# kanster/moped

Hardware: AMD Instinct MI355X
Metric: detections/sec (frames/s) 640x480 ~3k SIFT vs N models (higher is better)
Workload: dtype f32

## Files before the change

### include/moped_hip.h

```cpp
#ifndef MOPED_HIP_H
#define MOPED_HIP_H

#include <stddef.h>
#include <stdint.h>

#ifdef __cplusplus
extern "C" {
#endif

#define MH_DESC_DIM 128
#define MH_MAX_BATCH 32
#define MH_MAX_IMAGES 8
#define MH_MAX_MODELS 8192
#define MH_OK 0
#define MH_ERR_ARG (-1)
#define MH_ERR_HIP (-2)
#define MH_ERR_CAPACITY (-3)
#define MH_ERR_NODEVICE (-4)

typedef struct mh_ctx mh_ctx;


int mh_create(int device, mh_ctx** out);
void mh_destroy(mh_ctx* ctx);
// ... 35 lines not shown
int mh_match_stats(mh_ctx* ctx, int Q, uint32_t stats[4], int reset);
int mh_match_set_mode(mh_ctx* ctx, int mode);
int mh_pose_set_split(mh_ctx* ctx, int on);
int mh_match_launches(mh_ctx* ctx, uint32_t out[3]);
float mh_screen_margin(float qq, float dmax);
int mh_screen_values(mh_ctx* ctx, const float* q_host, int Q, int n_rows, float* out_host, float* dmax, float* spread,
                     int shape );
uint16_t mh_screen_record_value(float top, float thr);
void mh_screen_record_bounds(uint16_t value_bits, uint32_t row0, float tau, float spread, int N, float dmax, float* lo,
                             float* hi);
float mh_screen_pack_value(float v, uint32_t id, int bits);
float mh_screen_pack_pert(float qq, float dmax, int bits);
void mh_screen_sample_bounds(uint16_t value_bits, float tau, float pert, float dmax, float* lo, float* hi);
void mh_screen_launch_plan(int Q, int q_expected, int N, int32_t out[8]);
int mh_match_incomplete(mh_ctx* ctx, uint32_t* count, int reset);
int mh_screen_sample_values(mh_ctx* ctx, const float* q_host, int Q, const int32_t* row0_host, float* out_host);
int mh_match_query_candidates(mh_ctx* ctx, int Q, uint32_t* out);

int mh_match_local_dev(mh_ctx* ctx, const float* qn_dev, const float* qnorm_dev, int Q,
                       int32_t* idx1_dev, float* d1_dev, float* d2_dev);
int mh_match_local_counted_dev(mh_ctx* ctx, const float* qn_dev, const float* qnorm_dev, int Q,
                               const int32_t* q_count_dev, int q_expected, int32_t* idx1_dev, float* d1_dev,
                               float* d2_dev);
int mh_match_merge_dev(mh_ctx* ctx, const int32_t* idx1_s_dev, const float* d1_s_dev,
                       const float* d2_s_dev, int n_shards, int Q,
                       int32_t* idx1_dev, float* d1_dev, float* d2_dev);
int mh_normalize_dev(mh_ctx* ctx, float* q_dev, float* qnorm_dev, int Q);


int mh_meanshift(mh_ctx* ctx, const float* pts_host, int n, int dim, float radius,
// ... 387 lines not shown
```

### moped_amd/capi.py

```python
from __future__ import annotations

import ctypes as C
import os

import numpy as np

_HERE = os.path.dirname(os.path.abspath(__file__))
LIB_PATH = os.environ.get("MH_LIB_PATH") or os.path.join(_HERE, "libmoped_hip.so")

MH_OK = 0
MH_ERR_CAPACITY = -3


class MhError(RuntimeError):
    pass


class mh_corr(C.Structure):
    _fields_ = [("u", C.c_float), ("v", C.c_float), ("x", C.c_float), ("y", C.c_float), ("z", C.c_float)]


class mh_cam(C.Structure):
    _fields_ = [("K", C.c_float * 4), ("cam", C.c_float * 7)]

# ... 113 lines not shown
    "mh_db_upload_raw", "mh_db_share", "mh_match_stats", "mh_match_set_mode", "mh_match_launches", "mh_pose_set_split", "mh_frame_fetch_match_points", "mh_screen_margin", "mh_frame_counters", "mh_match_timing", "mh_frame_set_images", "mh_filter_images",
    "mh_pose_ransac_images",
    "mh_comm_unique_id", "mh_comm_create", "mh_comm_create_all", "mh_comm_create_host", "mh_comm_destroy", "mh_comm_info",
    "mh_frame_enqueue_sharded", "mh_frame_enqueue_sharded_batch", "mh_frame_enqueue_sharded_all",
    "mh_frame_previous_objects", "mh_frame_gather_objects", "mh_frame_enqueue_batch", "mh_frame_set_depth_image_batch",
    "mh_pose_kernel_info", "mh_db_upload_blocks", "mh_frame_fetch_matches_slot", "mh_frame_fetch_match_reps_slot",
    "mh_screen_values", "mh_screen_record_value", "mh_screen_record_bounds", "mh_reserve_batch", "mh_frame_run_host",
    "mh_frame_block_stride", "mh_frame_fetch_batch_async", "mh_frame_fetch_previous_async", "mh_frame_fetch_wait",
    "mh_frame_fetch_query", "mh_host_alloc", "mh_host_free", "mh_frame_run_host_begin", "mh_frame_wait_descriptors",
    "mh_step_match", "mh_step_match_fetch", "mh_step_cluster", "mh_step_pose", "mh_step_filter",
    "mh_set_linkage_scratch_limit",
    "mh_undistort_map", "mh_undistort", "mh_undistort_dev", "mh_frame_set_undistort",
    "mh_sift_extract_batch_dev", "mh_sift_debug_plan", "mh_sift_debug_level", "mh_sift_debug_candidates",
    "mh_sift_debug_keys", "mh_sift_debug_blur",
    "mh_screen_pack_value", "mh_screen_pack_pert", "mh_screen_sample_bounds", "mh_screen_launch_plan", "mh_match_incomplete",
    "mh_screen_sample_values", "mh_match_query_candidates",
    "mh_frame_enqueue_images", "mh_frame_enqueue_images_batch", "mh_frame_set_undistort_images", "mh_frame_image_counts",
    "mh_frame_features_image_dev",
    "mh_filter_depth_set_points", "mh_filter_depth", "mh_frame_set_filter_depth",
    "mh_frame_route", "mh_filter_depth_debug_form",
    "mh_depth_filter", "mh_depth_prop", "mh_frame_run_kinect_host",
    "mh_linkage_debug_matrix", "mh_linkage_debug_agglomerate", "mh_frame_debug_fetch_clusters_slot",
    "mh_planar_rows_dev", "mh_planar_rows_batch_dev", "mh_db_splice_image", "mh_db_splice_images",
    "mh_models_add_rows", "mh_models_write_xml",
]
COMM_ID_BYTES = 128
EX2_OBJECTS = 62
ALLGATHER_FN = C.CFUNCTYPE(C.c_int, C.c_void_p, C.c_void_p, C.c_void_p, C.c_size_t)

DIM = 128
DB_INSERT, DB_REPLACE, DB_REMOVE = 0, 1, 2
# ... 174 lines not shown
    L.mh_screen_record_bounds.argtypes = [C.c_uint16, C.c_uint32, f32, f32, i32, f32, C.POINTER(f32), C.POINTER(f32)]
    L.mh_screen_record_bounds.restype = None
    if hasattr(L, "mh_screen_pack_value"):
        L.mh_screen_pack_value.argtypes = [f32, C.c_uint32, i32]
        L.mh_screen_pack_value.restype = f32
        L.mh_screen_pack_pert.argtypes = [f32, f32, i32]
        L.mh_screen_pack_pert.restype = f32
        L.mh_screen_sample_bounds.argtypes = [C.c_uint16, f32, f32, f32, C.POINTER(f32), C.POINTER(f32)]
        L.mh_screen_sample_bounds.restype = None
        L.mh_screen_launch_plan.argtypes = [i32, i32, i32, vp]
        L.mh_screen_launch_plan.restype = None
        L.mh_match_incomplete.argtypes = [vp, C.POINTER(C.c_uint32), i32]
    if hasattr(L, "mh_screen_sample_values"):
        L.mh_screen_sample_values.argtypes = [vp, vp, i32, vp, vp]
        L.mh_match_query_candidates.argtypes = [vp, i32, vp]
    L.mh_db_upload_blocks.argtypes = [vp, vp, vp, vp, i32, i32, vp, vp, i32, i32]
    L.mh_frame_block_stride.argtypes = [i32]
    L.mh_frame_block_stride.restype = C.c_size_t
    L.mh_frame_fetch_batch_async.argtypes = [vp, i32, i32, vp, C.c_uint32]
    L.mh_frame_fetch_previous_async.argtypes = [vp, i32, vp, C.c_uint32]
    L.mh_frame_fetch_wait.argtypes = [vp, C.POINTER(C.c_int32)]
    L.mh_host_alloc.argtypes = [vp, C.c_size_t, C.POINTER(vp)]
    L.mh_host_free.argtypes = [vp, vp]
    L.mh_frame_wait_descriptors.argtypes = [vp]
    if hasattr(L, "mh_step_match"):
        L.mh_set_linkage_scratch_limit.argtypes = [vp, C.c_size_t]
        L.mh_step_match.argtypes = [vp, vp, vp, i32, C.POINTER(mh_cam), f32, i32]
        L.mh_step_match_fetch.argtypes = [vp, vp, vp, vp, i32, C.POINTER(C.c_int32)]
        L.mh_step_cluster.argtypes = [vp, f32, f32, i32, i32, vp, vp, vp, i32, i32, C.POINTER(C.c_int32)]
        L.mh_step_pose.argtypes = [vp, i32, C.POINTER(mh_pose_params), C.c_uint64, vp, i32, C.POINTER(C.c_int32)]
# ... 429 lines not shown
        st = np.zeros(4, np.uint32)
        self._ck(self.L.mh_match_stats(self.h, int(Q), _ptr(st), int(reset)), "mh_match_stats")
        return {"candidates": int(st[0]), "brute_force_queries": int(st[1]), "queries": int(st[2]),
                "two_stage": bool(st[3])}

    def match_query_candidates(self, Q):
        out = np.zeros(int(Q), np.uint32)
        self._ck(self.L.mh_match_query_candidates(self.h, int(Q), _ptr(out)), "mh_match_query_candidates")
        return out

    def match_incomplete(self, reset=False) -> int:
        n = C.c_uint32(0)
        self._ck(self.L.mh_match_incomplete(self.h, C.byref(n), int(reset)), "mh_match_incomplete")
        return int(n.value)

    def normalize(self, desc):
        d = np.ascontiguousarray(desc, np.float32).copy()
        self._ck(self.L.mh_normalize(self.h, _ptr(d), d.shape[0]), "mh_normalize")
        return d

    def match(self, q, ratio=0.8):
        q = np.ascontiguousarray(q, np.float32)
        Q = q.shape[0]
        acc = np.full(Q, -1, np.int32)
        raw = np.full(Q, -1, np.int32)
        d1 = np.zeros(Q, np.float32)
        d2 = np.zeros(Q, np.float32)
        self._ck(self.L.mh_match(self.h, _ptr(q), Q, ratio, _ptr(acc), _ptr(raw), _ptr(d1), _ptr(d2)), "mh_match")
        return acc, raw, d1, d2

# ... 935 lines not shown
```

### moped_amd/csrc/api.hip

```cpp
#include <algorithm>
#include <cmath>
#include <cstring>
#include <new>
#include <vector>

#include "context.h"
#include "steps.h"

using namespace mh;

namespace mh {

int use_stream(mh_ctx* ctx) {
  if (!ctx->held.empty()) db_poll_held(ctx, false);
  if (ctx->stream) return MH_OK;
  if (!ctx->own_stream) MH_HIP(ctx, hipStreamCreateWithFlags(&ctx->own_stream, hipStreamNonBlocking));
  ctx->stream = ctx->own_stream;
  return MH_OK;
}

int ensure_scratch(mh_ctx* ctx, size_t bytes) {
  if (bytes > ctx->scratch.cap) MH_HIP(ctx, ctx->scratch.ensure(bytes + bytes / 4 + 4096, ctx->stream));
  return MH_OK;
}
// ... 34 lines not shown
  MH_HIP(ctx, ctx->match_scratch.ensure(match_scratch_elems(Q, ctx->N > 0 ? ctx->N : 1), s));
  const int q_pad = screen_q_pad(Q);
  if (ctx->sdb.usable && q_pad > ctx->sbuf.q_pad) {
    ScreenBufs& b = ctx->sbuf;
    mh_ctx::ScreenOwn& o = ctx->screen_own;
    b = ScreenBufs();
    const size_t qp = (size_t)q_pad, slots = qp * screen_rec_slots();
    MH_HIP(ctx, o.qh.ensure(qp * DIM, s));
    MH_HIP(ctx, o.qbad.ensure(qp, s));
    MH_HIP(ctx, o.part.ensure(screen_part_bytes(q_pad), s));
    MH_HIP(ctx, o.tau.ensure(qp, s));
    MH_HIP(ctx, o.recs.ensure(slots, s));
    MH_HIP(ctx, o.ovf_cnt.ensure(qp, s));
    MH_HIP(ctx, o.ovf.ensure(qp * SCREEN_OVF_CAP, s));
    MH_HIP(ctx, o.stats.ensure(qp * 3, s));
    MH_HIP(ctx, o.inc.ensure(qp + 1, s));
    MH_HIP(ctx, hipMemsetAsync(o.inc, 0, (qp + 1) * sizeof(unsigned int), s));
    MH_HIP(ctx, hipMemsetAsync(o.recs, 0, slots * sizeof(uint2), s));
    MH_HIP(ctx, hipMemsetAsync(o.ovf_cnt, 0, qp * sizeof(int32_t), s));
    MH_HIP(ctx, hipMemsetAsync(o.stats, 0, qp * 3 * sizeof(unsigned int), s));
    b.qh = o.qh;
    b.qbad = o.qbad;
    b.part = reinterpret_cast<float2*>(o.part.p);
    b.tau = o.tau;
    b.recs = o.recs;
    b.ovf_cnt = o.ovf_cnt;
    b.ovf = o.ovf;
    b.stats = o.stats;
    b.inc = o.inc;
    b.ovf_cap = SCREEN_OVF_CAP;
    b.q_pad = q_pad;
  }
// ... 498 lines not shown

int mh_match_incomplete(mh_ctx* ctx, uint32_t* count, int reset) {
  if (!ctx || !count) return MH_ERR_ARG;
  MH_HIP(ctx, hipSetDevice(ctx->device));
  if (int rc_stream = mh::use_stream(ctx)) return rc_stream;
  MH_HIP(ctx, hipStreamSynchronize(ctx->stream));
  *count = 0;
  if (ctx->sbuf.inc) {
    unsigned int* c = ctx->sbuf.inc + ctx->sbuf.q_pad;
    MH_HIP(ctx, hipMemcpy(count, c, sizeof(unsigned int), hipMemcpyDeviceToHost));
    if (reset) MH_HIP(ctx, hipMemset(c, 0, sizeof(unsigned int)));
  }
  return MH_OK;
}

int mh_screen_values(mh_ctx* ctx, const float* q_host, int Q, int n_rows, float* out_host, float* dmax, float* spread,
                     int shape) {
  if (!ctx || !q_host || !out_host || Q <= 0 || n_rows <= 0 || (Q & 31) || (n_rows & 31)) {
    if (ctx) ctx->err = "mh_screen_values: Q and n_rows must be positive multiples of 32";
    return MH_ERR_ARG;
  }
  if (!ctx->sdb.dbh || n_rows > (ctx->N + 127) / 128 * 128) {
    ctx->err = "mh_screen_values: the database has no f16 image (fewer than 4096 rows?) or fewer rows than asked for";
    return MH_ERR_ARG;
  }
  MH_HIP(ctx, hipSetDevice(ctx->device));
  if (int rc_stream = mh::use_stream(ctx)) return rc_stream;
  const int q_pad = screen_q_pad(Q);
  hipStream_t s = ctx->stream;
  DevBuf<float> qd, qn, out;
// ... 150 lines not shown
```

### moped_amd/csrc/match_screen.hip

```cpp
#include <type_traits>
#include <hip/hip_fp16.h>

#include <algorithm>
#include <cstdlib>

#include "common.h"
#include "screen.h"

MH_TRACE_TU()

namespace mh {

namespace {

typedef _Float16 half8 __attribute__((ext_vector_type(8)));
typedef float v16f __attribute__((ext_vector_type(16)));
#define MH_AS1 __attribute__((address_space(1)))
#define MH_AS3 __attribute__((address_space(3)))

constexpr int SC_QPAD = 3 * 1024;
constexpr int SC_TILE = 128;
constexpr int SC_TILE_BYTES = SC_TILE * DIM * 2;
constexpr bool SC_SHAPE16_LARGE = true;
constexpr int SC_NW_LARGE = 8;
// ... 170 lines not shown
  const uint8_t* qbad;
  const int32_t* q_count;
  float2* part;
  float* part5;
  const float* tau;
  uint2* recs;
  int32_t* ovf_cnt;
  uint2* ovf;
  int Q, q_pad, ovf_cap, sub_cap;
  int n_sel, tile_first, tile_stride;
  int tiles_base, tiles_rem, n_splits;
  int n_splits_a;
  unsigned pack_keep;
  int skip_first, skip_stride;
  float dmax;
  int ablate;
};

__global__ void screen_tau_kernel(const float2* __restrict__ part, int n_splits_a, int q_pad, int Q,
                                  const int32_t* __restrict__ q_count, const float* __restrict__ qnorm,
                                  const uint8_t* __restrict__ qbad, float dmax, float* __restrict__ tau) {
  MH_TRACE_SCOPE(mh::TK_TAU);
  const int q = blockIdx.x * blockDim.x + threadIdx.x;
  if (q >= q_pad) return;
  const int Qe = q_count ? min(Q, *q_count) : Q;
  float t = __builtin_inff();
  if (q < Qe && !qbad[q]) {
    float B = -__builtin_inff(), S = -__builtin_inff();
    for (int s0 = 0; s0 < n_splits_a; s0 += 8) {
      float2 p[8];
// ... 443 lines not shown
    for (int nb = 0; nb < NQB; ++nb) {
      const float ob = __shfl_xor(b1[nb], 32), os = __shfl_xor(b2[nb], 32);
      const float S = fmaxf(fminf(b1[nb], ob), fmaxf(b2[nb], os));
      const float B = fmaxf(b1[nb], ob);
      const int q = q0 + nb * 32 + l32;
      if (half == 0 && q < A.q_pad) A.part[(size_t)split * A.q_pad + q] = make_float2(B, S);
    }
  }
}

typedef float v4f __attribute__((ext_vector_type(4)));
constexpr int SC_REC16_BYTES = 48;
constexpr int SC_RECBUF16 = 8 * 1024 / SC_REC16_BYTES;
constexpr int SC_LDS16_TAU = SC_LDS_TILES + 8 * SC_RECBUF16 * SC_REC16_BYTES;
constexpr int SC_LDS16_BYTES = SC_LDS16_TAU + 8 * 128 * 4;

template <int MODE, int NQB>
__global__ __launch_bounds__(512, 2) void screen16_kernel(const ScreenArgs A) {
  MH_TRACE_SCOPE(MODE == 0 ? mh::TK_PASS_A : mh::TK_PASS_B);
  constexpr int NW = 8;
  constexpr int QW = 32 * NQB;
  constexpr int QB = QW * NW;
  extern __shared__ __attribute__((aligned(16))) unsigned char lds[];
  const int tid = threadIdx.x;
  const int lane = tid & 63;
  const int wave = __builtin_amdgcn_readfirstlane(tid >> 6);
  const int quarter = lane >> 4, l16 = lane & 15;
  const unsigned lds_base = (unsigned)(uintptr_t)(MH_AS3 unsigned char*)lds;
  const int nqb = gridDim.x / A.n_splits;
  int qblock, split;
  {
    const int L = blockIdx.x, U = gridDim.x;
    const int x = L & 7, j = L >> 3;
    const int unit = x * (U >> 3) + min(x, U & 7) + j;
    split = unit / nqb;
// ... 13 lines not shown
    const int d = A.skip_stride - 1;
    if (sel_begin < A.skip_first) {
      tile_cur = sel_begin;
      gap_cur = A.skip_first - sel_begin;
    } else {
      const int jj = sel_begin - A.skip_first;
      tile_cur = sel_begin + 1 + jj / d;
      gap_cur = d - jj % d;
    }
  }
  auto stage = [&](int tile, int buf) {
    const unsigned char* tb = reinterpret_cast<const unsigned char*>(A.dbh) + (size_t)tile * SC_TILE_BYTES;
    const unsigned l = lds_base + buf * SC_TILE_BYTES + wave * 1024;
    dma16x4(voff, tb, tb + 8192, tb + 16384, tb + 24576, l, l + 8192, l + 16384, l + 24576);
    if (wave < 3)
      dma4(voff_dd, A.dneg + (size_t)tile * SC_DD, lds_base + SC_NBUF * SC_TILE_BYTES + buf * (SC_DD * 4) + wave * 256);
  };
  if (sel_begin < sel_end) stage(tile_cur, 0);
  half8 bq[NQB][2][4];
#pragma unroll
  for (int nb = 0; nb < NQB; ++nb)
#pragma unroll
    for (int tj = 0; tj < 2; ++tj) {
      const _Float16* row = A.qh + (size_t)(q0 + nb * 32 + 16 * tj + l16) * DIM + 8 * quarter;
#pragma unroll
      for (int s = 0; s < 4; ++s) bq[nb][tj][s] = *reinterpret_cast<const half8*>(row + 32 * s);
    }
  float pk[NQB][2][SC_PART5];
  unsigned n_rec[(NQB + 1) / 2] = {};
  float* const tau_lds = reinterpret_cast<float*>(lds + SC_LDS16_TAU) + wave * 128;
#pragma unroll
  for (int nb = 0; nb < NQB; ++nb)
#pragma unroll
    for (int tj = 0; tj < 2; ++tj)
#pragma unroll
      for (int k = 0; k < SC_PART5; ++k) pk[nb][tj][k] = -__builtin_inff();
  if (MODE == 1)
    for (int i = lane; i < QW; i += 64) tau_lds[i] = A.tau[q0 + i];
  __builtin_amdgcn_s_waitcnt(0x0F70);
  __syncthreads();

  uint4* const recbuf = reinterpret_cast<uint4*>(lds + SC_LDS_TILES + wave * (SC_RECBUF16 * SC_REC16_BYTES));
  int n_parked = 0;
  auto record_bits8 = [](const v4f& d0, const v4f& d1, float top, float thr) {
    unsigned bits = 0;
#pragma unroll
    for (int r = 3; r >= 0; --r) bits = __builtin_amdgcn_alignbit(bits, __float_as_uint(thr - d1[r]), 31);
#pragma unroll
    for (int r = 3; r >= 0; --r) bits = __builtin_amdgcn_alignbit(bits, __float_as_uint(thr - d0[r]), 31);
    return (bits & 0xFFu) | ((unsigned)screen_record_value(top, thr) << 16);
  };
  auto emit = [&](const v4f& d0, const v4f& d1, unsigned& nrec_word, int shift, int q, int row0, float top, float thr, int pos) {
    const int nrec = (int)((nrec_word >> shift) & 0xFFu);
    if (nrec < A.sub_cap) {
      const unsigned dst = (unsigned)q * SC_SLOT_PITCH + (4 * split + quarter) * A.sub_cap + nrec;
      nrec_word += 1u << shift;
      if (pos < SC_RECBUF16) {
        uint4* e = recbuf + 3 * pos;
        e[0] = make_uint4(dst, (unsigned)row0, __float_as_uint(thr), __float_as_uint(top));
        e[1] = make_uint4(__float_as_uint(d0[0]), __float_as_uint(d0[1]), __float_as_uint(d0[2]), __float_as_uint(d0[3]));
        e[2] = make_uint4(__float_as_uint(d1[0]), __float_as_uint(d1[1]), __float_as_uint(d1[2]), __float_as_uint(d1[3]));
      } else {
        A.recs[dst] = make_uint2((unsigned)row0 | SC_REC_LAYOUT16, record_bits8(d0, d1, top, thr));
      }
    } else {
      const int opos = atomicAdd(&A.ovf_cnt[q], 1);
      if (opos < A.ovf_cap) A.ovf[(size_t)q * A.ovf_cap + opos] = make_uint2((unsigned)row0 | SC_REC_LAYOUT16, record_bits8(d0, d1, top, thr));
      if (pos < SC_RECBUF16) recbuf[3 * pos] = make_uint4(0xFFFFFFFFu, 0u, 0u, 0u);
    }
  };
  auto emit_block = [&](bool hit0, bool hit1, const v4f (&p)[2][2], int nb, int row0, float m0, float m1, float thr0, float thr1) {
    const unsigned long long h0 = __ballot(hit0), h1 = __ballot(hit1);
    if ((h0 | h1) == 0ull) return;
    if (hit0)
      emit(p[0][0], p[1][0], n_rec[nb >> 1], 16 * (nb & 1), q0 + nb * 32 + l16, row0, m0, thr0,
           n_parked + (int)__builtin_amdgcn_mbcnt_hi((unsigned)(h0 >> 32), __builtin_amdgcn_mbcnt_lo((unsigned)h0, 0u)));
    n_parked += __popcll(h0);
    if (hit1)
      emit(p[0][1], p[1][1], n_rec[nb >> 1], 16 * (nb & 1) + 8, q0 + nb * 32 + 16 + l16, row0, m1, thr1,
           n_parked + (int)__builtin_amdgcn_mbcnt_hi((unsigned)(h1 >> 32), __builtin_amdgcn_mbcnt_lo((unsigned)h1, 0u)));
    n_parked += __popcll(h1);
  };
  auto flush_parked = [&]() {
    __builtin_amdgcn_fence(__ATOMIC_RELEASE, "wavefront");
    __builtin_amdgcn_wave_barrier();
    __builtin_amdgcn_fence(__ATOMIC_ACQUIRE, "wavefront");
    const int n = min(n_parked, SC_RECBUF16);
    for (int j = lane; j < n; j += 64) {
      const uint4 e = recbuf[3 * j];
      if (e.x == 0xFFFFFFFFu) continue;
      const uint4 x0 = recbuf[3 * j + 1], x1 = recbuf[3 * j + 2];
      const v4f d0 = {__uint_as_float(x0.x), __uint_as_float(x0.y), __uint_as_float(x0.z), __uint_as_float(x0.w)};
      const v4f d1 = {__uint_as_float(x1.x), __uint_as_float(x1.y), __uint_as_float(x1.z), __uint_as_float(x1.w)};
      A.recs[e.x] = make_uint2(e.y | SC_REC_LAYOUT16, record_bits8(d0, d1, __uint_as_float(e.w), __uint_as_float(e.z)));
    }
    __builtin_amdgcn_wave_barrier();
    n_parked = 0;
  };

  auto load_rb = [&](const unsigned char* T, int rb, half8 (&a)[2][4]) {
#pragma unroll
    for (int ti = 0; ti < 2; ++ti) {
// ... 21 lines not shown
        "v_max3_f32 %1, %1, %15, %16\n\t"
        "v_max3_f32 %0, %0, %2, %20\n\t"
        "v_max3_f32 %1, %1, %3, %20"
        : "=&v"(m0), "=&v"(m1), "=&v"(t0), "=&v"(t1)
        : "v"(acc[0][0][0]), "v"(acc[0][0][1]), "v"(acc[0][0][2]), "v"(acc[0][0][3]), "v"(acc[1][0][0]), "v"(acc[1][0][1]),
          "v"(acc[1][0][2]), "v"(acc[1][0][3]), "v"(acc[0][1][0]), "v"(acc[0][1][1]), "v"(acc[0][1][2]), "v"(acc[0][1][3]),
          "v"(acc[1][1][0]), "v"(acc[1][1][1]), "v"(acc[1][1][2]), "v"(acc[1][1][3]), "v"(floor));
  };
  auto max2 = [](float a, float b) {
    float r;
    asm("v_max_f32 %0, %1, %2" : "=v"(r) : "v"(a), "v"(b));
    return r;
  };

  int side = 0;
  const v4f ninf4 = {-__builtin_inff(), -__builtin_inff(), -__builtin_inff(), -__builtin_inff()};
  v4f pend[2][2] = {{ninf4, ninf4}, {ninf4, ninf4}};
  float pend_hi = 0.f;
  int pend_row0 = 0;
  const v4f zero4 = {0.f, 0.f, 0.f, 0.f};
  {
  MH_TRACE_PHASE(trace_loop_, MODE == 1 ? mh::TK_PASS_B_LOOP : mh::TK_PASS_A_LOOP);
  for (int sel = sel_begin; sel < sel_end; ++sel) {
    const bool more = sel + 1 < sel_end;
    int tile_nxt = tile_cur + (MODE == 0 ? A.tile_stride : 1), gap_nxt = gap_cur - 1;
    if (gap_nxt == 0) {
      tile_nxt += 1;
      gap_nxt = A.skip_stride - 1;
    }
    if (more) stage(tile_nxt, side ^ 1);
    const unsigned char* T = lds + side * SC_TILE_BYTES;
    const float* ddp = reinterpret_cast<const float*>(lds + SC_NBUF * SC_TILE_BYTES + side * (SC_DD * 4));
    const int row_tile = tile_cur * SC_TILE;
    tile_cur = tile_nxt;
    gap_cur = gap_nxt;
    if (!live) {
    } else if (MODE == 0) {
#pragma unroll 1
      for (int rb = 0; rb < SC_TILE / 32; ++rb) {
        half8 a[2][4];
        load_rb(T, rb, a);
        const unsigned blk = (unsigned)((sel - sel_begin) * 4 + rb) & ~A.pack_keep;
        v4f init[2];
#pragma unroll
        for (int ti = 0; ti < 2; ++ti) {
          const float4 v = *reinterpret_cast<const float4*>(ddp + rb * 32 + 16 * ti + 4 * quarter);
          init[ti] = v4f{v.x, v.y, v.z, v.w};
        }
#pragma unroll
        for (int nb = 0; nb < NQB; ++nb) {
          v4f acc[2][2] = {{init[0], init[0]}, {init[1], init[1]}};
// ... 14 lines not shown
#pragma unroll
            for (int k = SC_PART5 - 1; k > 0; --k) p[k] = __builtin_amdgcn_fmed3f(p[k - 1], p[k], m);
            p[0] = max2(p[0], m);
          }
          __builtin_amdgcn_sched_barrier(0);
        }
      }
    } else {
      const float4 hi4 = *reinterpret_cast<const float4*>(ddp + 128);
      const float hi[4] = {hi4.x, hi4.y, hi4.z, hi4.w};
#pragma unroll
      for (int rb = 0; rb < SC_TILE / 32; ++rb) {
        half8 a[2][4];
        load_rb(T, rb, a);
        const int row0 = row_tile + rb * 32 + 4 * quarter;
#pragma unroll
        for (int nb = 0; nb < NQB; ++nb) {
          const int pnb = (nb + NQB - 1) % NQB;
          v4f acc[2][2] = {{zero4, zero4}, {zero4, zero4}};
          float m0 = -__builtin_inff(), m1 = -__builtin_inff();
          const float t0 = tau_lds[pnb * 32 + l16], t1 = tau_lds[pnb * 32 + 16 + l16];
#pragma unroll
          for (int s = 0; s < 4; ++s) {
#pragma unroll
            for (int ti = 0; ti < 2; ++ti)
#pragma unroll
              for (int tj = 0; tj < 2; ++tj)
                acc[ti][tj] = __builtin_amdgcn_mfma_f32_16x16x32_f16(a[ti][s], bq[nb][tj][s], acc[ti][tj], 0, 0, 0);
            if (s == 2) m0 = max8(pend[0][0], pend[1][0]);
            if (s == 3) m1 = max8(pend[0][1], pend[1][1]);
          }
          __builtin_amdgcn_sched_group_barrier(0x008, 8, 0);
#pragma unroll
// ... 4 lines not shown
          __builtin_amdgcn_sched_barrier(0);
          {
            const float thr0 = t0 - pend_hi, thr1 = t1 - pend_hi;
            emit_block(m0 > thr0, m1 > thr1, pend, pnb, pend_row0, m0, m1, thr0, thr1);
          }
          __builtin_amdgcn_sched_barrier(0);
#pragma unroll
          for (int ti = 0; ti < 2; ++ti)
#pragma unroll
            for (int tj = 0; tj < 2; ++tj) pend[ti][tj] = acc[ti][tj];
          pend_row0 = row0;
          pend_hi = hi[rb];
        }
      }
    }
    if (more) asm volatile("s_waitcnt vmcnt(0)" ::: "memory");
    __syncthreads();
    side ^= 1;
  }
  }
  if (MODE == 1) {
    {
      const float m0 = max8(pend[0][0], pend[1][0]), m1 = max8(pend[0][1], pend[1][1]);
      const float thr0 = tau_lds[(NQB - 1) * 32 + l16] - pend_hi, thr1 = tau_lds[(NQB - 1) * 32 + 16 + l16] - pend_hi;
      emit_block(m0 > thr0, m1 > thr1, pend, NQB - 1, pend_row0, m0, m1, thr0, thr1);
    }
    flush_parked();
  }
  if (MODE == 0) {
#pragma unroll
    for (int nb = 0; nb < NQB; ++nb)
#pragma unroll
      for (int tj = 0; tj < 2; ++tj) {
        const int q = q0 + nb * 32 + 16 * tj + l16;
        if (q < A.q_pad) {
// ... 633 lines not shown
        p.Sb = c;
      }
    }
  }
  const int slots_target = n_tiles >= 2048 ? SC_SLOTS_MAX : (n_tiles >= 512 ? 160 : 96);
  p.sub_cap = std::max(1, std::min(std::max(3, (slots_target + 4 * p.Sb - 1) / (4 * p.Sb)), SC_SLOTS_MAX / (4 * p.Sb)));
  return p;
}

template <int NQB>
void launch_passes16(ScreenArgs a, int Q, int qe, int n_tiles, int sample, int blocks_a, int blocks_b, int* n_slots_out,
                     SampleGeom* geom_out, unsigned int* inc, hipEvent_t* ev, hipStream_t s) {
  constexpr int QB = 32 * NQB * 8;
  static DynLds attr0, attr1;
  attr0.ensure(screen16_kernel<0, NQB>, SC_LDS16_BYTES);
  attr1.ensure(screen16_kernel<1, NQB>, SC_LDS16_BYTES);
  const int nqb = (Q + QB - 1) / QB;
  const Plan16 p = plan_passes16<NQB>(qe, n_tiles, sample, blocks_a, blocks_b);
  a.n_sel = p.n_sel_a;
  a.tile_first = p.tile_first;
  a.tile_stride = p.stride;
  a.n_splits = p.Sa;
  a.tiles_base = p.n_sel_a / p.Sa;
  a.tiles_rem = p.n_sel_a % p.Sa;
  a.n_splits_a = p.Sa;
  a.pack_keep = ~((1u << p.pack_bits) - 1u);
  a.skip_first = a.skip_stride = 0;
  hipLaunchKernelGGL((screen16_kernel<0, NQB>), dim3(nqb * p.Sa), dim3(512), SC_LDS16_BYTES, s, a);
  if (ev) hipEventRecord(ev[2], s);
  SampleGeom g = {p.onesweep ? SC_SA_SLOTS : 0, p.pack_bits, a.tile_first, a.tile_stride, a.tiles_base, a.tiles_rem, a.n_sel};
  static_assert(SC_SA_SPLITS_MAX <= 2 * HO_PARTS_MAX, "a thread of screen_handover_kernel holds at most 8 lane slots");
// ... 4 lines not shown
    hipLaunchKernelGGL(screen_handover_kernel<8>, dim3((a.q_pad + 63) / 64), dim3(64, (p.Sa + 1) / 2), 0, s, (const float*)a.part5,
                       4 * p.Sa, a.q_pad, a.Q, a.q_count, a.qnorm, a.qbad, a.dmax, g, const_cast<float*>(a.tau), a.recs, inc);
#ifdef MH_EXPERIMENTS
  if (exp_int("MH_SCREEN_NO_HITS", 0)) hipMemsetAsync(const_cast<float*>(a.tau), 0x7f, (size_t)a.q_pad * sizeof(float), s);
#endif
  if (ev) hipEventRecord(ev[3], s);
  a.n_sel = p.n_sel_b;
  a.tile_first = 0;
  a.tile_stride = 1;
  a.skip_first = p.onesweep ? p.tile_first : 0;
  a.skip_stride = p.onesweep ? p.stride : 0;
  a.n_splits = p.Sb;
  a.tiles_base = p.n_sel_b / p.Sb;
  a.tiles_rem = p.n_sel_b % p.Sb;
  a.sub_cap = p.sub_cap;
  hipLaunchKernelGGL((screen16_kernel<1, NQB>), dim3(nqb * p.Sb), dim3(512), SC_LDS16_BYTES, s, a);
  if (ev) hipEventRecord(ev[4], s);
  *n_slots_out = 4 * p.Sb * a.sub_cap;
  *geom_out = g;
}

template <int WAVES, int PF>
void launch_pass_c(int grid, hipStream_t s, const RsArgs& args) {
  static DynLds attr;
  attr.ensure(rescore_kernel<WAVES, PF>, rs_lds_bytes(WAVES));
  hipLaunchKernelGGL((rescore_kernel<WAVES, PF>), dim3(grid), dim3(64 * WAVES), rs_lds_bytes(WAVES), s, args);
}

struct ShapeChoice {
  int nqb_sel;
  bool passes16;
};
ShapeChoice choose_shape(int qe, int n_tiles) {
  static const int nqb_pin = exp_int("MH_SCREEN_NQB", 0);
  int nqb_sel = qe > 640 ? 2 : 1;
  if (qe >= 2048 && (long)n_tiles * ((qe + 1023) / 1024) >= 16L * 256) nqb_sel = 4;
  if (nqb_pin >= 1 && nqb_pin <= 4) nqb_sel = nqb_pin;
  static const int shape_pin = exp_int("MH_SCREEN_SHAPE", 0);
  const bool shape16 = shape_pin == 2 || (shape_pin == 0 && SC_SHAPE16_LARGE);
  const bool p16 = shape16 && ((nqb_sel == 4 && (shape_pin == 2 || (qe + 1023) / 1024 >= 12)) || (nqb_sel == 2 && shape_pin == 2));
  return {nqb_sel, p16};
}

int screen_sample_every() {
  static const int sample = std::max(1, exp_int("MH_SCREEN_SAMPLE", 8));
  return sample;
}

}

void screen_launch_plan(int Q, int q_expected, int N, int out[8]) {
  const int qe = (q_expected > 0 && q_expected < Q) ? std::max(q_expected, std::min(Q, 256)) : Q;
  const int n_tiles = (N + SC_TILE - 1) / SC_TILE;
  for (int k = 0; k < 8; ++k) out[k] = 0;
  const ShapeChoice shape = choose_shape(qe, n_tiles);
  if (!shape.passes16) return;
  const int blocks_b = std::max(0, exp_int("MH_SCREEN_BLOCKS", 0)), blocks_a = std::max(1, exp_int("MH_SCREEN_BLOCKS_A", 256));
// ... 27 lines not shown
  a.qh = sb.qh;
  a.dbh = sdb.dbh;
  a.dneg = sdb.dneg;
  a.qnorm = qnorm;
  a.qbad = sb.qbad;
  a.q_count = q_count;
  a.part = sb.part;
  a.part5 = reinterpret_cast<float*>(sb.part);
  a.pack_keep = ~0u;
  a.skip_first = a.skip_stride = 0;
  a.tau = sb.tau;
  a.recs = sb.recs;
  a.ovf_cnt = sb.ovf_cnt;
  a.ovf = sb.ovf;
  a.ovf_cap = sb.ovf_cap;
  a.sub_cap = 1;
  a.Q = Q;
  a.q_pad = q_pad;
  a.dmax = sdb.dmax;
#ifdef SC_PROF
  a.ablate = g_sc_ablate;
#else
  a.ablate = 0;
#endif
  const ShapeChoice shape = choose_shape(qe, n_tiles);
  const int nqb_sel = shape.nqb_sel;
  int n_slots = 0;
  SampleGeom geom = {0, 0, 0, 1, 0, 0, 0};
  static const int nw_pin = exp_int("MH_SCREEN_NW", 0);
  const int nw_sel = nw_pin == 4 || nw_pin == 8 ? nw_pin : (nqb_sel == 4 ? SC_NW_LARGE : 8);
// ... 39 lines not shown
```

### moped_amd/csrc/screen.h

```cpp
#pragma once
#include <hip/hip_fp16.h>
#include <hip/hip_runtime.h>
#include <stdint.h>

namespace mh {

struct ScreenDb {
  const _Float16* dbh = nullptr;
  const float* dneg = nullptr;
  float dmax = 0.f;
  float spread = __builtin_inff();
  bool usable = false;
  int32_t zero_idx = -1;
  float zero_d1 = __builtin_inff(), zero_d2 = __builtin_inff();
};

struct ScreenBufs {
  _Float16* qh = nullptr;
  uint8_t* qbad = nullptr;
  float2* part = nullptr;
  float* tau = nullptr;
  uint2* recs = nullptr;
  int32_t* ovf_cnt = nullptr;
  uint2* ovf = nullptr;
// ... 52 lines not shown
size_t screen_rec_slots();

float screen_margin_host(float qq, float dmax);
void launch_screen_values(const _Float16* qh, int Q, const ScreenDb& sdb, int n_rows, float* out, hipStream_t s, int shape);
void launch_screen_sample_values(const float* qn, int Q, const ScreenDb& sdb, const int32_t* row0, float* out, hipStream_t s);
void launch_screen_prepare(const float* qn, const float* qnorm, int Q, int q_pad, _Float16* qh, uint8_t* qbad, hipStream_t s);
size_t screen_db_half_elems(int N);
size_t screen_dneg_elems(int N);
void launch_db_to_half(const float* db, const float* dnorm, int N, _Float16* dbh, float* dneg, unsigned int* stats,
                       hipStream_t s);
void launch_db_aggregates(const float* dnorm, int N, float* dneg, unsigned int* stats, hipStream_t s);
int screen_q_pad(int Q);
int screen_max_splits_a();
size_t screen_part_bytes(int q_pad);
void screen_launch_plan(int Q, int q_expected, int N, int out[8]);
bool screen_wanted(int q_expected, int N, int mode = -1);
void launch_match_screen(const float* qn, const float* qnorm, int Q, const float* db, const float* dnorm, int N,
                         const RowMap& rmap, const ScreenDb& sdb, const ScreenBufs& sb, int32_t* idx1, float* d1,
                         float* d2, hipStream_t s, const int32_t* q_count, int q_expected);

}
```

Measured before the change: 16690.

## Replace pass-B double buffer barrier with a three-slot LDS ring and per-wave counters

Pass B of the fp16 screen kernel now stages database tiles into a three-buffer LDS ring. Per-buffer ready and done counters, bumped by each wave's lane 0 with workgroup-scope atomics, replace the workgroup-wide __syncthreads at the end of every tile, so waves can drift apart instead of stalling on the slowest one. A bounded spin with a give-up path marks the affected queries as overflowed so the exact fallback handles them, and a counter plus an optional trace API expose how often that happens. The ring needs about 162 KB of LDS, which likely limits pass B to one workgroup per CU. It is used only when the selected tile count is at most 1024.

```diff
diff --git a/include/moped_hip.h b/include/moped_hip.h
--- a/include/moped_hip.h
+++ b/include/moped_hip.h
@@ -73,6 +73,7 @@
 void mh_screen_sample_bounds(uint16_t value_bits, float tau, float pert, float dmax, float* lo, float* hi);
 void mh_screen_launch_plan(int Q, int q_expected, int N, int32_t out[8]);
 int mh_match_incomplete(mh_ctx* ctx, uint32_t* count, int reset);
+int mh_screen_ring_stats(mh_ctx* ctx, uint64_t out[4], int reset);
 int mh_screen_sample_values(mh_ctx* ctx, const float* q_host, int Q, const int32_t* row0_host, float* out_host);
 int mh_match_query_candidates(mh_ctx* ctx, int Q, uint32_t* out);
 
diff --git a/moped_amd/capi.py b/moped_amd/capi.py
--- a/moped_amd/capi.py
+++ b/moped_amd/capi.py
@@ -151,7 +151,7 @@
     "mh_sift_extract_batch_dev", "mh_sift_debug_plan", "mh_sift_debug_level", "mh_sift_debug_candidates",
     "mh_sift_debug_keys", "mh_sift_debug_blur",
     "mh_screen_pack_value", "mh_screen_pack_pert", "mh_screen_sample_bounds", "mh_screen_launch_plan", "mh_match_incomplete",
-    "mh_screen_sample_values", "mh_match_query_candidates",
+    "mh_screen_sample_values", "mh_match_query_candidates", "mh_screen_ring_stats",
     "mh_frame_enqueue_images", "mh_frame_enqueue_images_batch", "mh_frame_set_undistort_images", "mh_frame_image_counts",
     "mh_frame_features_image_dev",
     "mh_filter_depth_set_points", "mh_filter_depth", "mh_frame_set_filter_depth",
@@ -356,6 +356,8 @@
     if hasattr(L, "mh_screen_sample_values"):
         L.mh_screen_sample_values.argtypes = [vp, vp, i32, vp, vp]
         L.mh_match_query_candidates.argtypes = [vp, i32, vp]
+    if hasattr(L, "mh_screen_ring_stats"):
+        L.mh_screen_ring_stats.argtypes = [vp, vp, i32]
     L.mh_db_upload_blocks.argtypes = [vp, vp, vp, vp, i32, i32, vp, vp, i32, i32]
     L.mh_frame_block_stride.argtypes = [i32]
     L.mh_frame_block_stride.restype = C.c_size_t
@@ -815,6 +817,11 @@
         self._ck(self.L.mh_match_incomplete(self.h, C.byref(n), int(reset)), "mh_match_incomplete")
         return int(n.value)
 
+    def screen_ring_stats(self, reset=False) -> dict:
+        out = np.zeros(4, np.uint64)
+        self._ck(self.L.mh_screen_ring_stats(self.h, _ptr(out), int(reset)), "mh_screen_ring_stats")
+        return {"giveups": int(out[0]), "wait_cycles": int(out[1]), "wavefronts": int(out[2]), "loop_cycles": int(out[3])}
+
     def normalize(self, desc):
         d = np.ascontiguousarray(desc, np.float32).copy()
         self._ck(self.L.mh_normalize(self.h, _ptr(d), d.shape[0]), "mh_normalize")
diff --git a/moped_amd/csrc/api.hip b/moped_amd/csrc/api.hip
--- a/moped_amd/csrc/api.hip
+++ b/moped_amd/csrc/api.hip
@@ -72,8 +72,8 @@
     MH_HIP(ctx, o.ovf_cnt.ensure(qp, s));
     MH_HIP(ctx, o.ovf.ensure(qp * SCREEN_OVF_CAP, s));
     MH_HIP(ctx, o.stats.ensure(qp * 3, s));
-    MH_HIP(ctx, o.inc.ensure(qp + 1, s));
-    MH_HIP(ctx, hipMemsetAsync(o.inc, 0, (qp + 1) * sizeof(unsigned int), s));
+    MH_HIP(ctx, o.inc.ensure(qp + 2, s));
+    MH_HIP(ctx, hipMemsetAsync(o.inc, 0, (qp + 2) * sizeof(unsigned int), s));
     MH_HIP(ctx, hipMemsetAsync(o.recs, 0, slots * sizeof(uint2), s));
     MH_HIP(ctx, hipMemsetAsync(o.ovf_cnt, 0, qp * sizeof(int32_t), s));
     MH_HIP(ctx, hipMemsetAsync(o.stats, 0, qp * 3 * sizeof(unsigned int), s));
@@ -602,6 +602,25 @@
   return MH_OK;
 }
 
+int mh_screen_ring_stats(mh_ctx* ctx, uint64_t out[4], int reset) {
+  if (!ctx || !out) return MH_ERR_ARG;
+  MH_HIP(ctx, hipSetDevice(ctx->device));
+  if (int rc_stream = mh::use_stream(ctx)) return rc_stream;
+  MH_HIP(ctx, hipStreamSynchronize(ctx->stream));
+  out[0] = 0;
+  if (ctx->sbuf.inc) {
+    unsigned int* c = ctx->sbuf.inc + ctx->sbuf.q_pad + 1;
+    unsigned int n = 0;
+    MH_HIP(ctx, hipMemcpy(&n, c, sizeof n, hipMemcpyDeviceToHost));
+    if (reset) MH_HIP(ctx, hipMemset(c, 0, sizeof n));
+    out[0] = n;
+  }
+  unsigned long long t[3];
+  screen_ring_trace(t, reset != 0);
+  for (int k = 0; k < 3; ++k) out[1 + k] = t[k];
+  return MH_OK;
+}
+
 int mh_screen_values(mh_ctx* ctx, const float* q_host, int Q, int n_rows, float* out_host, float* dmax, float* spread,
                      int shape) {
   if (!ctx || !q_host || !out_host || Q <= 0 || n_rows <= 0 || (Q & 31) || (n_rows & 31)) {
diff --git a/moped_amd/csrc/match_screen.hip b/moped_amd/csrc/match_screen.hip
--- a/moped_amd/csrc/match_screen.hip
+++ b/moped_amd/csrc/match_screen.hip
@@ -208,6 +208,7 @@
   unsigned pack_keep;
   int skip_first, skip_stride;
   float dmax;
+  unsigned int* giveup;
   int ablate;
 };
 
@@ -681,11 +682,30 @@
 constexpr int SC_RECBUF16 = 8 * 1024 / SC_REC16_BYTES;
 constexpr int SC_LDS16_TAU = SC_LDS_TILES + 8 * SC_RECBUF16 * SC_REC16_BYTES;
 constexpr int SC_LDS16_BYTES = SC_LDS16_TAU + 8 * 128 * 4;
-
-template <int MODE, int NQB>
+constexpr int SC_RING_NBUF = 3;
+constexpr int SC_RING_RECBUF = 149;
+constexpr int SC_RING_DD = SC_RING_NBUF * SC_TILE_BYTES;
+constexpr int SC_RING_TAU = SC_RING_DD + SC_RING_NBUF * SC_DD * 4;
+constexpr int SC_RING_REC = SC_RING_TAU + 8 * 128 * 4;
+constexpr int SC_RING_CNT = SC_RING_REC + 8 * SC_RING_RECBUF * SC_REC16_BYTES;
+constexpr int SC_RING_BYTES = SC_RING_CNT + 64;
+constexpr int SC_RING_TILES_MAX = 1024;
+constexpr unsigned SC_RING_SPINS = 1u << 22;
+static_assert(SC_RING_DD == 98304 && SC_RING_TAU == 100608 && SC_RING_REC == 104704 && SC_RING_CNT == 161920, "pass B's ring layout");
+static_assert(SC_RING_BYTES == 161984 && SC_RING_BYTES <= 160 * 1024, "three tiles, thresholds and hit buffers fit one workgroup's 160 KB");
+static_assert(SC_RING_REC % 16 == 0 && (SC_RING_RECBUF * SC_REC16_BYTES) % 16 == 0 && SC_RING_CNT % 16 == 0, "uint4 accesses");
+#ifdef MH_TRACE
+__device__ unsigned long long g_ring_trace[4];
+#endif
+
+template <int MODE, int NQB, bool RING = (MODE == 1)>
 __global__ __launch_bounds__(512, 2) void screen16_kernel(const ScreenArgs A) {
   MH_TRACE_SCOPE(MODE == 0 ? mh::TK_PASS_A : mh::TK_PASS_B);
+  static_assert(MODE == 1 || !RING, "the ring is pass B's");
   constexpr int NW = 8;
+  constexpr int NBUF = RING ? SC_RING_NBUF : SC_NBUF;
+  constexpr int OFF_DD = NBUF * SC_TILE_BYTES, OFF_TAU = RING ? SC_RING_TAU : SC_LDS16_TAU, OFF_REC = RING ? SC_RING_REC : SC_LDS_TILES;
+  constexpr int RECBUF = RING ? SC_RING_RECBUF : SC_RECBUF16;
   constexpr int QW = 32 * NQB;
   constexpr int QB = QW * NW;
   extern __shared__ __attribute__((aligned(16))) unsigned char lds[];
@@ -729,7 +749,7 @@
     const unsigned l = lds_base + buf * SC_TILE_BYTES + wave * 1024;
     dma16x4(voff, tb, tb + 8192, tb + 16384, tb + 24576, l, l + 8192, l + 16384, l + 24576);
     if (wave < 3)
-      dma4(voff_dd, A.dneg + (size_t)tile * SC_DD, lds_base + SC_NBUF * SC_TILE_BYTES + buf * (SC_DD * 4) + wave * 256);
+      dma4(voff_dd, A.dneg + (size_t)tile * SC_DD, lds_base + OFF_DD + buf * (SC_DD * 4) + wave * 256);
   };
   if (sel_begin < sel_end) stage(tile_cur, 0);
   half8 bq[NQB][2][4];
@@ -743,7 +763,7 @@
     }
   float pk[NQB][2][SC_PART5];
   unsigned n_rec[(NQB + 1) / 2] = {};
-  float* const tau_lds = reinterpret_cast<float*>(lds + SC_LDS16_TAU) + wave * 128;
+  float* const tau_lds = reinterpret_cast<float*>(lds + OFF_TAU) + wave * 128;
 #pragma unroll
   for (int nb = 0; nb < NQB; ++nb)
 #pragma unroll
@@ -752,10 +772,11 @@
       for (int k = 0; k < SC_PART5; ++k) pk[nb][tj][k] = -__builtin_inff();
   if (MODE == 1)
     for (int i = lane; i < QW; i += 64) tau_lds[i] = A.tau[q0 + i];
+  if (RING && tid < 16) reinterpret_cast<unsigned*>(lds + SC_RING_CNT)[tid] = tid == 0 ? 8u : 0u;
   __builtin_amdgcn_s_waitcnt(0x0F70);
   __syncthreads();
 
-  uint4* const recbuf = reinterpret_cast<uint4*>(lds + SC_LDS_TILES + wave * (SC_RECBUF16 * SC_REC16_BYTES));
+  uint4* const recbuf = reinterpret_cast<uint4*>(lds + OFF_REC + wave * (RECBUF * SC_REC16_BYTES));
   int n_parked = 0;
   auto record_bits8 = [](const v4f& d0, const v4f& d1, float top, float thr) {
     unsigned bits = 0;
@@ -770,7 +791,7 @@
     if (nrec < A.sub_cap) {
       const unsigned dst = (unsigned)q * SC_SLOT_PITCH + (4 * split + quarter) * A.sub_cap + nrec;
       nrec_word += 1u << shift;
-      if (pos < SC_RECBUF16) {
+      if (pos < RECBUF) {
         uint4* e = recbuf + 3 * pos;
         e[0] = make_uint4(dst, (unsigned)row0, __float_as_uint(thr), __float_as_uint(top));
         e[1] = make_uint4(__float_as_uint(d0[0]), __float_as_uint(d0[1]), __float_as_uint(d0[2]), __float_as_uint(d0[3]));
@@ -781,7 +802,7 @@
     } else {
       const int opos = atomicAdd(&A.ovf_cnt[q], 1);
       if (opos < A.ovf_cap) A.ovf[(size_t)q * A.ovf_cap + opos] = make_uint2((unsigned)row0 | SC_REC_LAYOUT16, record_bits8(d0, d1, top, thr));
-      if (pos < SC_RECBUF16) recbuf[3 * pos] = make_uint4(0xFFFFFFFFu, 0u, 0u, 0u);
+      if (pos < RECBUF) recbuf[3 * pos] = make_uint4(0xFFFFFFFFu, 0u, 0u, 0u);
     }
   };
   auto emit_block = [&](bool hit0, bool hit1, const v4f (&p)[2][2], int nb, int row0, float m0, float m1, float thr0, float thr1) {
@@ -800,7 +821,7 @@
     __builtin_amdgcn_fence(__ATOMIC_RELEASE, "wavefront");
     __builtin_amdgcn_wave_barrier();
     __builtin_amdgcn_fence(__ATOMIC_ACQUIRE, "wavefront");
-    const int n = min(n_parked, SC_RECBUF16);
+    const int n = min(n_parked, RECBUF);
     for (int j = lane; j < n; j += 64) {
       const uint4 e = recbuf[3 * j];
       if (e.x == 0xFFFFFFFFu) continue;
@@ -852,6 +873,43 @@
   };
 
   int side = 0;
+  int ring_round = 0;
+  bool computing = live, polling = true;
+  unsigned seen_ready = 8u, seen_done = 0u;
+#ifdef MH_TRACE
+  unsigned long long t_wait = 0;
+  const unsigned long long t_loop0 = __builtin_amdgcn_s_memtime();
+#endif
+  auto ring_word = [&](int k) { return reinterpret_cast<unsigned*>(lds + SC_RING_CNT) + k; };
+  auto ring_peek = [&](int k) { return *reinterpret_cast<volatile unsigned*>(ring_word(k)); };
+  auto ring_signal = [&](int k) {
+    if (lane == 0) __hip_atomic_fetch_add(ring_word(k), 1u, __ATOMIC_RELAXED, __HIP_MEMORY_SCOPE_WORKGROUP);
+  };
+  auto ring_give_up = [&]() {
+    computing = polling = false;
+    for (int i = lane; i < QB; i += 64)
+      if (qblock * QB + i < Qe) atomicAdd(&A.ovf_cnt[qblock * QB + i], A.ovf_cap + 1);
+    if (lane == 0 && A.giveup) atomicAdd(A.giveup, 1u);
+  };
+  auto ring_wait = [&](int k, unsigned need, unsigned seen) {
+    if (seen < need && polling) {
+#ifdef MH_TRACE
+      const unsigned long long t0 = __builtin_amdgcn_s_memtime();
+#endif
+      for (unsigned spins = 0;; ++spins) {
+        if (__builtin_amdgcn_readfirstlane(ring_peek(k)) >= need) break;
+        if (spins == SC_RING_SPINS) {
+          ring_give_up();
+          break;
+        }
+        __builtin_amdgcn_s_sleep(1);
+      }
+#ifdef MH_TRACE
+      t_wait += __builtin_amdgcn_s_memtime() - t0;
+#endif
+    }
+    asm volatile("" ::: "memory");
+  };
   const v4f ninf4 = {-__builtin_inff(), -__builtin_inff(), -__builtin_inff(), -__builtin_inff()};
   v4f pend[2][2] = {{ninf4, ninf4}, {ninf4, ninf4}};
   float pend_hi = 0.f;
@@ -866,13 +924,31 @@
       tile_nxt += 1;
       gap_nxt = A.skip_stride - 1;
     }
-    if (more) stage(tile_nxt, side ^ 1);
+    const int side_nxt = RING ? (side == 2 ? 0 : side + 1) : side ^ 1;
+    const int round_nxt = ring_round + (side == 2 ? 1 : 0);
+    if (RING) {
+      if (more) {
+        ring_wait(4 + side_nxt, 8u * (unsigned)round_nxt, seen_done);
+        stage(tile_nxt, side_nxt);
+      }
+      if (computing) ring_wait(side, 8u * (unsigned)(ring_round + 1), seen_ready);
+      seen_ready = seen_done = 0u;
+    } else {
+      if (more) stage(tile_nxt, side_nxt);
+    }
     const unsigned char* T = lds + side * SC_TILE_BYTES;
-    const float* ddp = reinterpret_cast<const float*>(lds + SC_NBUF * SC_TILE_BYTES + side * (SC_DD * 4));
+    const float* ddp = reinterpret_cast<const float*>(lds + OFF_DD + side * (SC_DD * 4));
     const int row_tile = tile_cur * SC_TILE;
     tile_cur = tile_nxt;
     gap_cur = gap_nxt;
-    if (!live) {
+    if (!computing) {
+      if (RING) {
+        if (more) {
+          asm volatile("s_waitcnt vmcnt(0)" ::: "memory");
+          ring_signal(side_nxt);
+        }
+        ring_signal(4 + side);
+      }
     } else if (MODE == 0) {
 #pragma unroll 1
       for (int rb = 0; rb < SC_TILE / 32; ++rb) {
@@ -917,9 +993,26 @@
         half8 a[2][4];
         load_rb(T, rb, a);
         const int row0 = row_tile + rb * 32 + 4 * quarter;
+        unsigned early_ready = 0u, early_done = 0u;
 #pragma unroll
         for (int nb = 0; nb < NQB; ++nb) {
           const int pnb = (nb + NQB - 1) % NQB;
+          if (RING && rb == 2 && nb == 1 && more) {
+            asm volatile("s_waitcnt vmcnt(0)" ::: "memory");
+            ring_signal(side_nxt);
+          }
+          if (RING && rb == 3 && nb == 1) {
+            asm volatile("s_waitcnt lgkmcnt(0)" ::: "memory");
+            ring_signal(4 + side);
+          }
+          if (RING && rb == 3 && nb == NQB - 2 && more) {
+            early_ready = ring_peek(side_nxt);
+            early_done = ring_peek(4 + (side_nxt == 2 ? 0 : side_nxt + 1));
+          }
+          if (RING && rb == 3 && nb == NQB - 1 && more) {
+            seen_ready = __builtin_amdgcn_readfirstlane(early_ready);
+            seen_done = __builtin_amdgcn_readfirstlane(early_done);
+          }
           v4f acc[2][2] = {{zero4, zero4}, {zero4, zero4}};
           float m0 = -__builtin_inff(), m1 = -__builtin_inff();
           const float t0 = tau_lds[pnb * 32 + l16], t1 = tau_lds[pnb * 32 + 16 + l16];
@@ -954,11 +1047,29 @@
         }
       }
     }
-    if (more) asm volatile("s_waitcnt vmcnt(0)" ::: "memory");
-    __syncthreads();
-    side ^= 1;
-  }
-  }
+    if (RING) {
+      side = side_nxt;
+      ring_round = round_nxt;
+    } else {
+      if (more) asm volatile("s_waitcnt vmcnt(0)" ::: "memory");
+#ifdef MH_TRACE
+      const unsigned long long t0 = __builtin_amdgcn_s_memtime();
+#endif
+      __syncthreads();
+#ifdef MH_TRACE
+      t_wait += __builtin_amdgcn_s_memtime() - t0;
+#endif
+      side = side_nxt;
+    }
+  }
+  }
+#ifdef MH_TRACE
+  if (MODE == 1 && lane == 0 && live) {
+    atomicAdd(&g_ring_trace[0], t_wait);
+    atomicAdd(&g_ring_trace[1], 1ull);
+    atomicAdd(&g_ring_trace[2], __builtin_amdgcn_s_memtime() - t_loop0);
+  }
+#endif
   if (MODE == 1) {
     {
       const float m0 = max8(pend[0][0], pend[1][0]), m1 = max8(pend[0][1], pend[1][1]);
@@ -1622,7 +1733,7 @@
   constexpr int QB = 32 * NQB * 8;
   static DynLds attr0, attr1;
   attr0.ensure(screen16_kernel<0, NQB>, SC_LDS16_BYTES);
-  attr1.ensure(screen16_kernel<1, NQB>, SC_LDS16_BYTES);
+  attr1.ensure(screen16_kernel<1, NQB>, SC_RING_BYTES);
   const int nqb = (Q + QB - 1) / QB;
   const Plan16 p = plan_passes16<NQB>(qe, n_tiles, sample, blocks_a, blocks_b);
   a.n_sel = p.n_sel_a;
@@ -1657,7 +1768,18 @@
   a.tiles_base = p.n_sel_b / p.Sb;
   a.tiles_rem = p.n_sel_b % p.Sb;
   a.sub_cap = p.sub_cap;
-  hipLaunchKernelGGL((screen16_kernel<1, NQB>), dim3(nqb * p.Sb), dim3(512), SC_LDS16_BYTES, s, a);
+  bool ring = p.n_sel_b <= SC_RING_TILES_MAX;
+#ifdef MH_EXPERIMENTS
+  static const int ring_pin = exp_int("MH_SCREEN_RING", -1);
+  if (ring_pin == 0 || ring_pin == 1) ring = ring_pin == 1;
+#endif
+  if (!ring) {
+    static DynLds attr1b;
+    attr1b.ensure(screen16_kernel<1, NQB, false>, SC_LDS16_BYTES);
+    hipLaunchKernelGGL((screen16_kernel<1, NQB, false>), dim3(nqb * p.Sb), dim3(512), SC_LDS16_BYTES, s, a);
+  } else {
+    hipLaunchKernelGGL((screen16_kernel<1, NQB>), dim3(nqb * p.Sb), dim3(512), SC_RING_BYTES, s, a);
+  }
   if (ev) hipEventRecord(ev[4], s);
   *n_slots_out = 4 * p.Sb * a.sub_cap;
   *geom_out = g;
@@ -1684,6 +1806,25 @@
   const bool p16 = shape16 && ((nqb_sel == 4 && (shape_pin == 2 || (qe + 1023) / 1024 >= 12)) || (nqb_sel == 2 && shape_pin == 2));
   return {nqb_sel, p16};
 }
+
+}
+
+void screen_ring_trace(unsigned long long out[3], bool reset) {
+  out[0] = out[1] = out[2] = 0;
+#ifdef MH_TRACE
+  unsigned long long v[4] = {};
+  if (hipMemcpyFromSymbol(v, HIP_SYMBOL(g_ring_trace), sizeof v) == hipSuccess)
+    for (int k = 0; k < 3; ++k) out[k] = v[k];
+  if (reset) {
+    const unsigned long long z[4] = {};
+    (void)hipMemcpyToSymbol(HIP_SYMBOL(g_ring_trace), z, sizeof z);
+  }
+#else
+  (void)reset;
+#endif
+}
+
+namespace {
 
 int screen_sample_every() {
   static const int sample = std::max(1, exp_int("MH_SCREEN_SAMPLE", 8));
@@ -1741,6 +1882,7 @@
   a.ovf_cnt = sb.ovf_cnt;
   a.ovf = sb.ovf;
   a.ovf_cap = sb.ovf_cap;
+  a.giveup = sb.inc ? sb.inc + sb.q_pad + 1 : nullptr;
   a.sub_cap = 1;
   a.Q = Q;
   a.q_pad = q_pad;
diff --git a/moped_amd/csrc/screen.h b/moped_amd/csrc/screen.h
--- a/moped_amd/csrc/screen.h
+++ b/moped_amd/csrc/screen.h
@@ -90,6 +90,7 @@
 int screen_max_splits_a();
 size_t screen_part_bytes(int q_pad);
 void screen_launch_plan(int Q, int q_expected, int N, int out[8]);
+void screen_ring_trace(unsigned long long out[3], bool reset);
 bool screen_wanted(int q_expected, int N, int mode = -1);
 void launch_match_screen(const float* qn, const float* qnorm, int Q, const float* db, const float* dnorm, int N,
                          const RowMap& rmap, const ScreenDb& sdb, const ScreenBufs& sb, int32_t* idx1, float* d1,
```

After: 16820, median of 6. About the same (+0.8%).
